# liamscarlett/slate-d35

Measured on AMD Instinct MI355X. Metric: fp64 TFLOP/s (whole node) for dgemm / dpotrf / dgetrf / dgeqrf, n=64k, at 1/2/4/8 MI355X, higher is better.
Workload: dtype fp64

## Files before the change

### csrc/include/slate_amd/local_blas.hh

```
#pragma once

#include <string>
#include <utility>
#include <vector>

#include "types.hh"
#include "comm.hh"
#include "device.hh"

namespace slate {
namespace lb {

struct Ctx {
    Target target = Target::HostTask;
    hipStream_t stream = nullptr;
    bool dev() const { return target == Target::Devices; }
    Loc loc() const { return dev() ? Loc::Device : Loc::Host; }
    static Ctx host() { return Ctx{Target::HostTask, nullptr}; }
    static Ctx device(int queue) { return Ctx{Target::Devices, device::queue(queue)}; }
    Ctx on(int queue) const { return dev() ? device(queue) : *this; }
};

class Scratch {
public:
// ... 42 lines not shown

constexpr int64_t kSkinnyRhs = 16;

template <typename T>
void gemv(Ctx const& c, Op opA, int64_t m, int64_t k, int64_t nr, T alpha, T const* A, int64_t lda, T const* X,
          int64_t ldx, T beta, T* Y, int64_t ldy);

template <typename T>
void gemm_tri(Ctx const& c, Uplo uplo, Op opA, Op opB, int64_t n, int64_t k, T alpha,
              T const* A, int64_t lda, T const* B, int64_t ldb, T beta, T* C, int64_t ldc);

template <typename T>
void herk(Ctx const& c, Uplo uplo, Op op, int64_t n, int64_t k, real_type<T> alpha,
          T const* A, int64_t lda, real_type<T> beta, T* C, int64_t ldc);
template <typename T>
void syrk(Ctx const& c, Uplo uplo, Op op, int64_t n, int64_t k, T alpha,
          T const* A, int64_t lda, T beta, T* C, int64_t ldc);
template <typename T>
void her2k(Ctx const& c, Uplo uplo, Op op, int64_t n, int64_t k, T alpha, T const* A, int64_t lda,
           T const* B, int64_t ldb, real_type<T> beta, T* C, int64_t ldc);
template <typename T>
void syr2k(Ctx const& c, Uplo uplo, Op op, int64_t n, int64_t k, T alpha, T const* A, int64_t lda,
           T const* B, int64_t ldb, T beta, T* C, int64_t ldc);
template <typename T>
void hemm(Ctx const& c, Side side, Uplo uplo, int64_t m, int64_t n, T alpha, T const* A, int64_t lda,
          T const* B, int64_t ldb, T beta, T* C, int64_t ldc, bool hermitian = true);
template <typename T>
void trsm(Ctx const& c, Side side, Uplo uplo, Op op, Diag diag, int64_t m, int64_t n, T alpha,
          T const* A, int64_t lda, T* B, int64_t ldb);
template <typename T>
// ... 59 lines not shown
```

### csrc/include/slate_amd/slate.hh

```
#pragma once

#include "enums.hh"
#include "types.hh"
#include "exception.hh"
#include "util.hh"
#include "device.hh"
#include "comm.hh"
#include "grid.hh"
#include "matrix.hh"
#include "inproc.hh"
#include "func.hh"
#include "method.hh"
#include "matgen.hh"
#include "init.hh"
#include "eig_host.hh"
#include "debug.hh"

#include <vector>

namespace slate {

template <typename T>
using TriangularFactors = std::vector<Matrix<T>>;

// ... 311 lines not shown
GebrdStats gebrd_stats();

template <typename T>
void geqp3(Matrix<T>& A, std::vector<int64_t>& jpvt, TriangularFactors<T>& T_, Options const& opts = {});
template <typename T>
void unmqr_geqp3(Side side, Op op, Matrix<T>& A, TriangularFactors<T>& T_, Matrix<T>& C, Options const& opts = {});
template <typename T>
int64_t gelsy(Matrix<T>& A, Matrix<T>& BX, real_type<T> rcond, Options const& opts = {});
struct Geqp3Stats {
    int64_t columns = 0, panels = 0, host_syncs = 0, norm_recomputes = 0;
    int64_t launches_norms = 0, launches_pivot = 0, launches_swap = 0, launches_column = 0, launches_larfg = 0,
            launches_product = 0, launches_finish = 0, launches_recompute = 0;
    double ms_pivot = 0, ms_product = 0, ms_panel = 0, ms_gemm = 0, ms_larft = 0;
};
Geqp3Stats geqp3_stats();

template <typename T>
void syev(SymmetricMatrix<T>& A, std::vector<real_type<T>>& Lambda, Matrix<T>& Z, Options const& opts = {});
template <typename T>
void sygst(int64_t itype, SymmetricMatrix<T>& A, SymmetricMatrix<T> const& B, Options const& opts = {});
template <typename T>
void sygv(int64_t itype, SymmetricMatrix<T>& A, SymmetricMatrix<T>& B, std::vector<real_type<T>>& Lambda,
          Matrix<T>& Z, Options const& opts = {});
template <typename T>
int64_t sytrf(SymmetricMatrix<T>& A, std::vector<int64_t>& ipiv, Options const& opts = {});
template <typename T>
void sytrs(SymmetricMatrix<T> const& A, std::vector<int64_t> const& ipiv, Matrix<T>& B, Options const& opts = {});
template <typename T>
int64_t sysv(SymmetricMatrix<T>& A, std::vector<int64_t>& ipiv, Matrix<T>& B, Options const& opts = {});
template <typename T>
// ... 23 lines not shown
```

### csrc/kernels/gemm_mfma.hip

```cpp
#include "device_common.hh"
#include "kernels.hh"

#include <cstdarg>
#include <cstdio>
#include <cstdlib>
#include <type_traits>

#ifndef GEMM_SPLIT
#define GEMM_SPLIT 1
#endif
#ifndef GEMM_JB
#define GEMM_JB 2
#endif
#ifndef GEMM_ROT
#define GEMM_ROT true
#endif

namespace slate_amd {
namespace dev {

namespace {
std::atomic<GemmVariantCounter*> g_variant_head{nullptr};
}
GemmVariantCounter::GemmVariantCounter(const char* fmt, ...) {
// ... 450 lines not shown
{
    if (m <= 0 || n <= 0 || batch <= 0) return;
    bool a_kc = (transA != 'N'), b_kc = (transB == 'N');
    if (a_kc && b_kc)
        launch_gemm<T, true, true>(m, n, k, alpha, A, lda, sA, B, ldb, sB, beta, C, ldc, sC, batch, stream);
    else if (a_kc)
        launch_gemm<T, true, false>(m, n, k, alpha, A, lda, sA, B, ldb, sB, beta, C, ldc, sC, batch, stream);
    else if (b_kc)
        launch_gemm<T, false, true>(m, n, k, alpha, A, lda, sA, B, ldb, sB, beta, C, ldc, sC, batch, stream);
    else
        launch_gemm<T, false, false>(m, n, k, alpha, A, lda, sA, B, ldb, sB, beta, C, ldc, sC, batch, stream);
}

template <typename T>
void gemm_tri_real(char uplo, char transA, char transB, int64_t n, int64_t k,
                   T alpha, const T* A, int64_t lda, const T* B, int64_t ldb,
                   T beta, T* C, int64_t ldc, hipStream_t stream)
{
    if (n <= 0) return;
    bool a_kc = (transA != 'N'), b_kc = (transB == 'N');
#define SLATE_TRI_LAUNCH(U)                                                                   \
    if (a_kc && b_kc) launch_gemm<T, true, true, U>(n, n, k, alpha, A, lda, 0, B, ldb, 0, beta, C, ldc, 0, 1, stream); \
    else if (a_kc)    launch_gemm<T, true, false, U>(n, n, k, alpha, A, lda, 0, B, ldb, 0, beta, C, ldc, 0, 1, stream); \
    else if (b_kc)    launch_gemm<T, false, true, U>(n, n, k, alpha, A, lda, 0, B, ldb, 0, beta, C, ldc, 0, 1, stream); \
    else              launch_gemm<T, false, false, U>(n, n, k, alpha, A, lda, 0, B, ldb, 0, beta, C, ldc, 0, 1, stream);
    if (uplo == 'L') { SLATE_TRI_LAUNCH('L') }
    else { SLATE_TRI_LAUNCH('U') }
#undef SLATE_TRI_LAUNCH
}

template <typename T>
void gemm_stair_real(int64_t m, int64_t n, int64_t k, T alpha, const T* A, int64_t lda, const T* B, int64_t ldb,
                     StairMap const& sm, T beta, T* C, int64_t ldc, hipStream_t stream)
{
    if (m <= 0 || n <= 0) return;
    constexpr int VEC = 16 / sizeof(T);
    auto al = [](const void* p) { return (reinterpret_cast<uintptr_t>(p) % 16) == 0; };
    bool aligned = al(A) && al(B) && (lda % VEC == 0) && (ldb % VEC == 0) && sm.nb % VEC == 0;
    launch_tile<T, false, false, 'S', 128, 128>(m, n, k, alpha, A, lda, 0, B, ldb, 0, beta, C, ldc, 0, 1,
                                                aligned, stream, sm);
// ... 19 lines not shown
        s2 += p[(b + 2) * mn];
        s3 += p[(b + 3) * mn];
    }
    for (; b < splits; ++b) s0 += p[b * mn];
    T s = (s0 + s1) + (s2 + s3);
    T* c = C + i + j * ldc;
    *c = (beta == T(0)) ? alpha * s : alpha * s + beta * (*c);
}

template <typename T>
void splitk_reduce(int64_t m, int64_t n, int splits, const T* P, T alpha, T beta, T* C, int64_t ldc, hipStream_t s) {
    if (m <= 0 || n <= 0) return;
    dim3 grid((unsigned)((m + 255) / 256), (unsigned)n);
    hipLaunchKernelGGL(splitk_reduce_kernel<T>, grid, dim3(256), 0, s, m, n, splits, P, alpha, beta, C, ldc);
}
template void splitk_reduce<double>(int64_t, int64_t, int, const double*, double, double, double*, int64_t, hipStream_t);
template void splitk_reduce<float>(int64_t, int64_t, int, const float*, float, float, float*, int64_t, hipStream_t);

template void gemm_tri_real<double>(char, char, char, int64_t, int64_t, double, const double*, int64_t,
                                    const double*, int64_t, double, double*, int64_t, hipStream_t);
template void gemm_tri_real<float>(char, char, char, int64_t, int64_t, float, const float*, int64_t,
                                   const float*, int64_t, float, float*, int64_t, hipStream_t);

template void gemm_real<double>(char, char, int64_t, int64_t, int64_t, double, const double*, int64_t, int64_t,
                                const double*, int64_t, int64_t, double, double*, int64_t, int64_t, int64_t, hipStream_t);
template void gemm_real<float>(char, char, int64_t, int64_t, int64_t, float, const float*, int64_t, int64_t,
                               const float*, int64_t, int64_t, float, float*, int64_t, int64_t, int64_t, hipStream_t);

}
}
```

### csrc/kernels/kernels.hh

```
#pragma once

#include <hip/hip_runtime_api.h>
#include <atomic>
#include <cstdint>
#include "dev_types.hh"
#include "matgen_entry.hh"
#include "slate_amd/secular.hh"
#include "slate_amd/sturm.hh"

namespace slate_amd {
namespace dev {

template <typename T> using rt = typename real_type_t<T>::type;

struct RowDist {
    int64_t row0;
    int64_t mb;
    int64_t lrow_begin;
    int p, rsrc, myrow, rrel;
};
SLATE_HD inline int rd_owner(RowDist const& d, int64_t gr) { return int(((d.row0 + gr) / d.mb + d.rsrc) % d.p); }
SLATE_HD inline int64_t rd_lrow(RowDist const& d, int64_t gr) {
    int64_t R = d.row0 + gr;
    return (R / d.mb / d.p) * d.mb + R % d.mb - d.lrow_begin;
// ... 261 lines not shown
struct GemmVariantCounter {
    char name[56];
    std::atomic<uint64_t> count{0};
    GemmVariantCounter* next = nullptr;
    explicit GemmVariantCounter(const char* fmt, ...) __attribute__((format(printf, 2, 3)));
    void hit() { count.fetch_add(1, std::memory_order_relaxed); }
};
void gemm_variant_counts(void (*fn)(const char* name, uint64_t count, void* arg), void* arg);
template <typename T>
void gemm_real(char transA, char transB, int64_t m, int64_t n, int64_t k,
               T alpha, const T* A, int64_t lda, int64_t sA,
               const T* B, int64_t ldb, int64_t sB,
               T beta, T* C, int64_t ldc, int64_t sC, int64_t batch, hipStream_t stream);
template <typename T>
void gemm_tri_real(char uplo, char transA, char transB, int64_t n, int64_t k,
                   T alpha, const T* A, int64_t lda, const T* B, int64_t ldb,
                   T beta, T* C, int64_t ldc, hipStream_t stream);
template <typename T>
void splitk_reduce(int64_t m, int64_t n, int splits, const T* P, T alpha, T beta, T* C, int64_t ldc, hipStream_t s);
struct StairMap {
    const int64_t* btab = nullptr;
    int64_t c0 = 0, r0 = 0;
    int nb = 0, p = 1, q = 1, prow = 0, pcol = 0;
};
template <typename T>
void gemm_stair_real(int64_t m, int64_t n, int64_t k, T alpha, const T* A, int64_t lda, const T* B, int64_t ldb,
                     StairMap const& sm, T beta, T* C, int64_t ldc, hipStream_t stream);
void gemm_bf16s(int nsplit, char uplo, char transA, char transB, int64_t m, int64_t n, int64_t k,
                float alpha, const float* A, int64_t lda, const float* B, int64_t ldb,
                float beta, float* C, int64_t ldc, hipStream_t stream);
template <typename T>
void gemm_cplx(char uplo, char transA, char transB, int64_t m, int64_t n, int64_t k,
               T alpha, const T* A, int64_t lda, const T* B, int64_t ldb,
               T beta, T* C, int64_t ldc, hipStream_t stream);
// ... 112 lines not shown
```

### csrc/python/bind.cc

```cpp
#include <pybind11/pybind11.h>
#include <chrono>
#include <thread>
#include <pybind11/numpy.h>
#include <pybind11/stl.h>
#include <pybind11/functional.h>

#include "slate_amd/slate.hh"
#include "../src/lu_dist.hh"
#include "slate_amd/trace.hh"
#include "slate_amd/runtime.hh"
#include "slate_amd/inproc.hh"
#include "bind_drivers.hh"
#include <pybind11/numpy.h>

#include <algorithm>
#include <cmath>
#include <complex>
#include <chrono>
#include <cstring>

namespace py = pybind11;
using namespace slate;

class PyHostComm : public HostComm {
// ... 562 lines not shown
        r["host_syncs"] = st.host_syncs;
        r["launches_column"] = st.launches_column;
        r["launches_larfg_u"] = st.launches_larfg_u;
        r["launches_pass1"] = st.launches_pass1;
        r["launches_finish_y"] = st.launches_finish_y;
        r["launches_larfg_v"] = st.launches_larfg_v;
        r["launches_pass2"] = st.launches_pass2;
        r["launches_finish_x"] = st.launches_finish_x;
        r["ms_pass1"] = st.ms_pass1;
        r["ms_pass2"] = st.ms_pass2;
        r["ms_panel"] = st.ms_panel;
        r["ms_gemm"] = st.ms_gemm;
        r["ms_larft"] = st.ms_larft;
        return r;
    });
    m.def("geqp3_stats", []() {
        const Geqp3Stats st = geqp3_stats();
        py::dict r;
        r["columns"] = st.columns;
        r["panels"] = st.panels;
        r["host_syncs"] = st.host_syncs;
        r["norm_recomputes"] = st.norm_recomputes;
        r["launches_norms"] = st.launches_norms;
        r["launches_pivot"] = st.launches_pivot;
        r["launches_swap"] = st.launches_swap;
        r["launches_column"] = st.launches_column;
        r["launches_larfg"] = st.launches_larfg;
        r["launches_product"] = st.launches_product;
        r["launches_finish"] = st.launches_finish;
        r["launches_recompute"] = st.launches_recompute;
// ... 186 lines not shown
```

### csrc/python/bind_drivers.hh

```
#pragma once

#include <pybind11/pybind11.h>
#include <pybind11/stl.h>
#include "slate_amd/slate.hh"
#include "slate_amd/local_blas.hh"
#include "slate_amd/eig_host.hh"
#include <pybind11/numpy.h>

namespace py = pybind11;

slate::Options to_options(py::dict d);

inline int& ops_queue() { static int q = 0; return q; }

template <typename T>
void bind_drivers(py::module_& m, std::string const& s) {
    using namespace slate;
    using R = real_type<T>;
    using G = py::call_guard<py::gil_scoped_release>;
    auto O = [](py::dict d) { return to_options(d); };
    (void)O;
#define DEF(name, ...) m.def((std::string(name) + "_" + s).c_str(), __VA_ARGS__)

    DEF("gemm", [](T a, Matrix<T> const& A, Matrix<T> const& B, T b, Matrix<T>& C, py::dict o) {
// ... 365 lines not shown
    });
    DEF("lb_gemm", [=](std::string ta, std::string tb, int64_t mm, int64_t n, int64_t k, T a, uintptr_t A, int64_t lda,
                       uintptr_t B, int64_t ldb, T b, uintptr_t C, int64_t ldc) {
        py::gil_scoped_release r;
        auto c = dctx();
        lb::gemm<T>(c, cop(ta), cop(tb), mm, n, k, a, (T*)A, lda, (T*)B, ldb, b, (T*)C, ldc);
        dsync(c);
    });
    DEF("lb_herk", [=](std::string up, std::string op, int64_t n, int64_t k, R a, uintptr_t A, int64_t lda, R b,
                       uintptr_t C, int64_t ldc) {
        py::gil_scoped_release r;
        auto c = dctx();
        lb::herk<T>(c, cup(up), cop(op), n, k, a, (T*)A, lda, b, (T*)C, ldc);
        dsync(c);
    });
    DEF("lb_gemm_tri", [=](std::string up, std::string ta, std::string tb, int64_t n, int64_t k, T a, uintptr_t A,
                           int64_t lda, uintptr_t B, int64_t ldb, T b, uintptr_t C, int64_t ldc) {
        py::gil_scoped_release r;
        auto c = dctx();
        lb::gemm_tri<T>(c, cup(up), cop(ta), cop(tb), n, k, a, (T*)A, lda, (T*)B, ldb, b, (T*)C, ldc);
        dsync(c);
    });
    DEF("lb_trsm", [=](std::string sd, std::string up, std::string op, std::string dg, int64_t mm, int64_t n, T a,
                       uintptr_t A, int64_t lda, uintptr_t B, int64_t ldb) {
        py::gil_scoped_release r;
        auto c = dctx();
        lb::trsm<T>(c, sd == "L" ? Side::Left : Side::Right, cup(up), cop(op), dg == "U" ? Diag::Unit : Diag::NonUnit,
                    mm, n, a, (T*)A, lda, (T*)B, ldb);
        dsync(c);
    });
// ... 69 lines not shown
```

### csrc/src/local_blas.cc

```cpp
#include "slate_amd/local_blas.hh"
#include "slate_amd/host_blas.hh"
#include "../kernels/kernels.hh"
#include "slate_amd/eig_host.hh"

#include <atomic>
#include <map>
#include <mutex>
#include <cstring>
#include <cstdlib>

namespace slate {
namespace lb {

using slate_amd::dev::dptr;
using slate_amd::dev::dval;
namespace kd = slate_amd::dev;

namespace {

struct Arena {
    struct Chunk { char* p; size_t size; };
    std::vector<Chunk> chunks;
    size_t cur = 0;
    size_t off = 0;
// ... 223 lines not shown
            return;
        }
        static const int64_t kchunk = [] {
            const char* e = std::getenv("SLATE_GEMM_KCHUNK");
            return e ? std::max<int64_t>(0, std::atoll(e)) : int64_t(0);
        }();
        const bool chunk = kchunk > 0 && k > kchunk && m * n >= int64_t(4096) * 4096;
        for (int64_t k0 = 0; k0 < std::max<int64_t>(k, 1); k0 += chunk ? kchunk : std::max<int64_t>(k, 1)) {
            const int64_t kk = chunk ? std::min(kchunk, k - k0) : k;
            T const* Ak = A + (ta == 'N' ? k0 * lda : k0);
            T const* Bk = B + (tb == 'N' ? k0 : k0 * ldb);
            const T bk = k0 == 0 ? beta : T(1);
            if (uplo == 'G') kd::gemm_real<T>(ta, tb, m, n, kk, alpha, Ak, lda, 0, Bk, ldb, 0, bk, C, ldc, 0, 1, s);
            else {
                slate_assert(m == n);
                kd::gemm_tri_real<T>(uplo, ta, tb, n, kk, alpha, Ak, lda, Bk, ldb, bk, C, ldc, s);
            }
        }
    } else {
        kd::gemm_cplx(uplo, opc(opA), opc(opB), m, n, k, dval(alpha), dptr(A), lda, dptr(B), ldb,
                      dval(beta), dptr(C), ldc, s);
    }
}

template <typename T>
void dset(hipStream_t s, char uplo, int64_t m, int64_t n, T off, T diag, T* A, int64_t lda) {
    kd::geset(uplo, m, n, dval(off), dval(diag), dptr(A), lda, s);
}

template <typename T>
void dcopy(hipStream_t s, int64_t m, int64_t n, T const* A, int64_t lda, T* B, int64_t ldb) {
// ... 73 lines not shown
void real_diag(Ctx const& c, int64_t n, T* C, int64_t ldc) {
    if constexpr (is_complex_v<T>)
        kd::gen_diag('R', 0.0, n, n, dptr(C), ldc, n, 1, 0, 0, 0, n, 1, 0, 0, 0, c.stream);
}
}

template <typename T>
void herk(Ctx const& c, Uplo uplo, Op op, int64_t n, int64_t k, real_type<T> alpha,
          T const* A, int64_t lda, real_type<T> beta, T* C, int64_t ldc) {
    if (n <= 0) return;
    if (!c.dev()) { host::rankk(true, uplo, op, n, k, T(alpha), A, lda, T(beta), C, ldc); return; }
    Op o1 = op == Op::NoTrans ? Op::NoTrans : Op::ConjTrans;
    Op o2 = op == Op::NoTrans ? Op::ConjTrans : Op::NoTrans;
    gemm_tri(c, uplo, o1, o2, n, k, T(alpha), A, lda, A, lda, T(beta), C, ldc);
    real_diag(c, n, C, ldc);
}

template <typename T>
void syrk(Ctx const& c, Uplo uplo, Op op, int64_t n, int64_t k, T alpha,
          T const* A, int64_t lda, T beta, T* C, int64_t ldc) {
    if (n <= 0) return;
    if (!c.dev()) { host::rankk(false, uplo, op, n, k, alpha, A, lda, beta, C, ldc); return; }
    Op o1 = op == Op::NoTrans ? Op::NoTrans : Op::Trans;
    Op o2 = op == Op::NoTrans ? Op::Trans : Op::NoTrans;
    gemm_tri(c, uplo, o1, o2, n, k, alpha, A, lda, A, lda, beta, C, ldc);
}

template <typename T>
void her2k(Ctx const& c, Uplo uplo, Op op, int64_t n, int64_t k, T alpha, T const* A, int64_t lda,
           T const* B, int64_t ldb, real_type<T> beta, T* C, int64_t ldc) {
// ... 781 lines not shown
void copy2d(Ctx const& c, int64_t m, int64_t n, T const* src, int64_t lds, T* dst, int64_t ldd) {
    if (m <= 0 || n <= 0) return;
    if (!c.dev()) {
        for (int64_t j = 0; j < n; ++j) std::memcpy(dst + j * ldd, src + j * lds, m * sizeof(T));
        return;
    }
    device::memcpy2d_async(dst, ldd * sizeof(T), src, lds * sizeof(T), m * sizeof(T), n, c.stream);
}

#define SLATE_LB_INST(T)                                                                                   \
    template void gemm<T>(Ctx const&, Op, Op, int64_t, int64_t, int64_t, T, T const*, int64_t, T const*, int64_t, T, T*, int64_t); \
    template void gemm_tri<T>(Ctx const&, Uplo, Op, Op, int64_t, int64_t, T, T const*, int64_t, T const*, int64_t, T, T*, int64_t); \
    template void gemv<T>(Ctx const&, Op, int64_t, int64_t, int64_t, T, T const*, int64_t, T const*, int64_t, T, T*, int64_t); \
    template void gemm_splitk<T>(Ctx const&, Op, Op, int64_t, int64_t, int64_t, int64_t, T, T const*, int64_t, T const*, int64_t, T, T*, int64_t); \
    template void herk<T>(Ctx const&, Uplo, Op, int64_t, int64_t, real_type<T>, T const*, int64_t, real_type<T>, T*, int64_t); \
    template void syrk<T>(Ctx const&, Uplo, Op, int64_t, int64_t, T, T const*, int64_t, T, T*, int64_t);  \
    template void her2k<T>(Ctx const&, Uplo, Op, int64_t, int64_t, T, T const*, int64_t, T const*, int64_t, real_type<T>, T*, int64_t); \
    template void syr2k<T>(Ctx const&, Uplo, Op, int64_t, int64_t, T, T const*, int64_t, T const*, int64_t, T, T*, int64_t); \
    template void hemm<T>(Ctx const&, Side, Uplo, int64_t, int64_t, T, T const*, int64_t, T const*, int64_t, T, T*, int64_t, bool); \
    template void trsm<T>(Ctx const&, Side, Uplo, Op, Diag, int64_t, int64_t, T, T const*, int64_t, T*, int64_t); \
    template void trmm<T>(Ctx const&, Side, Uplo, Op, Diag, int64_t, int64_t, T, T const*, int64_t, T*, int64_t); \
    template void potrf<T>(Ctx const&, Uplo, int64_t, T*, int64_t, int*, int64_t);                        \
    template void trtri<T>(Ctx const&, Uplo, Diag, int64_t, T*, int64_t);                                 \
    template void trtri_to<T>(Ctx const&, Uplo, Diag, int64_t, T const*, int64_t, T*, int64_t);           \
    template void lauum<T>(Ctx const&, Uplo, int64_t, T*, int64_t);                                        \
    template void getrf_panel<T>(Ctx const&, int64_t, int64_t, T*, int64_t, int64_t*, int64_t*, int*, int64_t, bool, bool, double); \
    template void apply_perm<T>(Ctx const&, int64_t, int64_t const*, int64_t const*, int64_t, T*, int64_t); \
    template void geqrf_panel<T>(Ctx const&, int64_t, int64_t, T*, int64_t, T*, T*, int64_t);             \
    template void larfb<T>(Ctx const&, Side, Op, int64_t, int64_t, int64_t, T const*, int64_t, T const*, int64_t, T*, int64_t); \
    template void form_v<T>(Ctx const&, int64_t, int64_t, T const*, int64_t, T*, int64_t);                \
// ... 54 lines not shown
```

### csrc/src/qr.cc

```cpp
#include "internal.hh"
#include "spread.hh"
#include "lu_dist.hh"

#include <cstdlib>

namespace slate {

using namespace internal;

namespace {

inline int64_t qr_kchunk() {
    static int64_t v = [] {
        const char* e = std::getenv("SLATE_QR_KCHUNK");
        return e ? std::atoll(e) : int64_t(8192);
    }();
    return v;
}

template <typename T>
struct TsqrPanel {
    static constexpr int maxr = 8;
    int64_t nb;
    Work<T> Tloc, Rcur, Rrecv, Ecur, Etmp, Qloc, LUb, Ytmp, Dg, Tw, sgn, taul, Gq;
    Work<int> cq_flag;
    Work<double> cq_ssq;
    int* cq_host = nullptr;
    bool cholqr_on = false;
    std::vector<Work<T>> Sst, Ttt;
    const int64_t tSel = Sched::tok(30, 0);

    TsqrPanel(Target target, int np, int64_t nb_, int64_t max_rows, bool single_cholqr = false) : nb(nb_) {
        if (np <= 1 && !single_cholqr) return;
// ... 22 lines not shown
    TsqrPanel(TsqrPanel const&) = delete;
    TsqrPanel& operator=(TsqrPanel const&) = delete;

    bool cholqr(Sched& S, int qP, Comm& cm, T* ap, int64_t lda, int64_t mr, int64_t kb, int64_t M, int64_t tPan,
                bool shifted) {
        using R = real_type<T>;
        const double u = double(std::numeric_limits<R>::epsilon()) / 2;
        const double shift = 11.0 * (double(M) * double(kb) + double(kb) * double(kb + 1)) * u;
        const Op cT = is_complex_v<T> ? Op::ConjTrans : Op::Trans;
        S.task(qP, {tPan}, {tSel}, [&, ap, mr, kb, shift, shifted, cT](lb::Ctx const& c) {
            trace::Block t2("geqrf_cholqr");
            using DT = slate_amd::dev::dev_t<T>;
            const int64_t ldq = std::max<int64_t>(mr, 1);
            int* dflag = cq_flag.data();
            const int npass = shifted ? 3 : 2;
            lb::copy2d(c, mr, kb, ap, lda, Qloc.data(), ldq);
            if (c.dev()) device::memset_async(dflag + 1, 0, sizeof(int), c.stream);
            else dflag[1] = 0;
            for (int pass = 0; pass < npass; ++pass) {
                T* G = Gq.data();
                lb::herk(c, Uplo::Lower, Op::ConjTrans, kb, mr, R(1), Qloc.data(), ldq, R(0), G, kb);
                cm.allreduce(G, size_t(kb * kb), ReduceOp::Sum, c.loc(), c.stream);
                const bool sh = shifted && pass == 0, chk = pass == npass - 1;
                if (c.dev()) {
                    if (sh) slate_amd::dev::cholqr_shift<DT>(slate_amd::dev::dptr(G), kb, int(kb), shift, c.stream);
                    if (chk)
                        slate_amd::dev::cholqr_check<DT>(slate_amd::dev::dptr(G), kb, int(kb), 0.5, dflag,
                                                         cq_ssq.data(), c.stream);
                } else if (sh) {
                    R tr = 0;
                    for (int64_t i = 0; i < kb; ++i) tr += std::real(G[i + i * kb]);
                    for (int64_t i = 0; i < kb; ++i) G[i + i * kb] += T(R(shift) * tr);
                } else if (chk) {
                    double ssq = 0;
                    for (int64_t j = 0; j < kb; ++j)
                        for (int64_t i = j; i < kb; ++i) {
                            const double d = double(std::abs(G[i + j * kb] - (i == j ? T(1) : T(0))));
                            ssq += (i == j ? 1.0 : 2.0) * d * d;
                        }
                    dflag[0] = (ssq <= 0.25) ? 0 : 1;
                }
                lb::potrf(c, Uplo::Lower, kb, G, kb, dflag + 1, 0);
                lb::trsm(c, Side::Right, Uplo::Lower, cT, Diag::NonUnit, mr, kb, T(1), G, kb, Qloc.data(), ldq);
                if (pass == 0) {
                    lb::set(c, Uplo::General, kb, kb, T(0), T(0), Rcur.data(), kb);
                    lb::copy<T, T>(c, Uplo::Upper, cT, kb, kb, G, kb, Rcur.data(), kb);
                } else {
                    lb::trmm(c, Side::Left, Uplo::Lower, cT, Diag::NonUnit, kb, kb, T(1), G, kb, Rcur.data(), kb);
                }
            }
            if (c.dev()) device::memcpy_async(cq_host, dflag, 2 * sizeof(int), c.stream);
        });
        if (dev_) slate_hip_call(hipStreamSynchronize(S.ctx(qP).stream));
        return cq_host[0] == 0 && cq_host[1] == 0;
    }

    void enqueue(Sched& S, int qP, Comm& cm, int root, int me, std::vector<int64_t> const& rows_r, T* ap,
                 int64_t lda, int64_t mr, int64_t kb, int64_t kd, T* Tk, int64_t tPan, int64_t tP) {
        int64_t Mtot = 0;
        for (auto r : rows_r) Mtot += r;
        if (cholqr_on && kd == kb && Mtot >= 2 * kb &&
            (cholqr(S, qP, cm, ap, lda, mr, kb, Mtot, tPan, false) ||
             cholqr(S, qP, cm, ap, lda, mr, kb, Mtot, tPan, true))) {
            reconstruct(S, qP, cm, root, me, ap, lda, mr, kb, kd, Tk, tPan, tP);
            return;
        }
        tree(S, qP, cm, root, me, rows_r, ap, lda, mr, kb, kd, tPan);
        reconstruct(S, qP, cm, root, me, ap, lda, mr, kb, kd, Tk, tPan, tP);
    }

    void tree(Sched& S, int qP, Comm& cm, int root, int me, std::vector<int64_t> const& rows_r, T* ap,
              int64_t lda, int64_t mr, int64_t kb, int64_t kd, int64_t tPan) {
        const int p = int(rows_r.size());
        const int pk = root;
        const bool diag = (me == root);
        const int myrow = me;
        Comm& colF = cm;
        std::vector<int> part;
        for (int d = 0; d < p; ++d) { int r = (pk + d) % p; if (rows_r[r] > 0) part.push_back(r); }
        const int np = int(part.size());
        std::vector<int64_t> cnt(np);
        for (int i = 0; i < np; ++i) cnt[i] = std::min(rows_r[part[i]], kb);
        int ix = -1;
// ... 83 lines not shown
                S.task(qP, {}, {tSel}, [&, r_, ms, kd](lb::Ctx const& c) {
                    lb::copy2d(c, r_.mine, kd, Etmp.data(), ms, Ecur.data(), r_.mine);
                });
                ecnt = r_.mine;
            }
            S.task(qP, {tSel}, {tSel}, [&, ap, mr, rr, kd, ecnt](lb::Ctx const& c) {
                trace::Block t2("geqrf_tsqr_qlocal");
                lb::set(c, Uplo::General, mr, kd, T(0), T(0), Qloc.data(), mr);
                lb::copy2d(c, ecnt, kd, Ecur.data(), ecnt, Qloc.data(), mr);
                lb::larfb(c, Side::Left, Op::NoTrans, mr, kd, rr, ap, lda, Tloc.data(), nb, Qloc.data(), mr);
            });
        }
    }

    void reconstruct(Sched& S, int qP, Comm& cm, int root, int me, T* ap, int64_t lda, int64_t mr, int64_t kb,
                     int64_t kd, T* Tk, int64_t tPan, int64_t tP) {
        const int pk = root;
        const bool diag = (me == root);
        Comm& colF = cm;
        if (diag) {
            S.task(qP, {tSel}, {tSel}, [&, mr, kd](lb::Ctx const& c) {
                trace::Block t2("geqrf_tsqr_hr_lu");
                lb::add(c, Uplo::General, kd, kd, T(-1), Qloc.data(), mr, T(0), LUb.data(), kd);
                internal::ludist::lu_sign(c, kd, LUb.data(), kd, sgn.data());
            });
        }
        S.task(qP, {}, {tSel}, [&, kd, pk](lb::Ctx const& c) {
            trace::Block t2("geqrf_tsqr_bcast_lu");
            bcast(colF, LUb.data(), size_t(kd * kd), pk, c);
            bcast(colF, sgn.data(), size_t(kd), pk, c);
        });
        const int64_t off = diag ? kd : 0, nbelow = std::max<int64_t>(mr - off, 0);
        S.task(qP, {tSel}, {tPan, tSel}, [&, ap, mr, kd, off, nbelow](lb::Ctx const& c) {
            trace::Block t2("geqrf_tsqr_hr_v");
            lb::trsm(c, Side::Right, Uplo::Upper, Op::NoTrans, Diag::NonUnit, nbelow, kd, T(-1), LUb.data(), kd,
                     Qloc.data() + off, std::max<int64_t>(mr, 1));
            lb::copy2d(c, nbelow, kd, Qloc.data() + off, std::max<int64_t>(mr, 1), ap + off, lda);
        });
        if (diag) {
            S.task(qP, {tSel}, {tPan, tSel, tP}, [&, ap, kb, kd, Tk](lb::Ctx const& c) {
                trace::Block t2("geqrf_tsqr_hr_t");
                lb::set(c, Uplo::General, kd, kd, T(0), T(0), Dg.data(), kd);
                lb::copy2d(c, int64_t(1), kd, sgn.data(), int64_t(1), Dg.data(), kd + 1);
                lb::gemm(c, Op::NoTrans, Op::NoTrans, kd, kb, kd, T(1), Dg.data(), kd, Rcur.data(), kd, T(0), ap,
                         lda);
                lb::copy2d(c, kd, kd, LUb.data(), kd, Ytmp.data(), kd);
                lb::set(c, Uplo::Upper, kd, kd, T(0), T(0), Ytmp.data(), kd);
                lb::add(c, Uplo::Lower, kd, kd, T(1), Ytmp.data(), kd, T(1), ap, lda);
                lb::set(c, Uplo::General, kd, kd, T(0), T(0), Tw.data(), kd);
                lb::copy<T, T>(c, Uplo::Upper, Op::NoTrans, kd, kd, LUb.data(), kd, Tw.data(), kd);
                lb::set(c, Uplo::General, kb, kb, T(0), T(0), Tk, kb);
// ... 10 lines not shown
    const int p = g.p(), q = g.q(), myrow = g.myrow(), mycol = g.mycol();
    const Loc loc = loc_of(target);
    const int64_t mt = A.mt(), nt = A.nt(), m = A.m();
    const int64_t kt = std::min(mt, nt);
    const int64_t nb = A.nb();
    LocalBlock<T> L = A.local(loc, true);
    T* a = L.ptr;
    const int64_t lda = L.ld, mloc = L.m, nloc = L.n;
    LocalBlock<T> LT = Tf.local(loc, true);
    T* tm = LT.ptr;
    const int64_t ldt = LT.ld;
    const int qC = device::kCommQueue, qP = 1;
    Comm& colF = g.col_fast();
    Comm& rowF = g.row_fast();

    Sched S(target);
    const int R = int(std::max<int64_t>(2, la + 2));
    std::vector<Work<T>> WV(R), WT(R), WW(R), WW2(R), Wtau(R);
    for (int r = 0; r < R; ++r) {
        WV[r].resize(target, size_t(std::max<int64_t>(mloc, 1)) * nb);
        WT[r].resize(target, size_t(nb) * nb);
        WW[r].resize(target, size_t(nb) * std::max<int64_t>(nloc, 1));
        WW2[r].resize(target, size_t(nb) * std::max<int64_t>(nloc, 1));
        Wtau[r].resize(target, size_t(nb));
    }
    static const bool cq1_env = [] {
        const char* e = std::getenv("SLATE_QR_CHOLQR1");
        return !e || std::atoi(e) != 0;
    }();
    const bool cq1 = p == 1 && cq1_env && target == Target::Devices && nb >= 256 && A.m() >= 16384;
// ... 247 lines not shown
            trace::Block t2("unmqr_allreduce");
            if (mC > 0) g.row().allreduce(W, W, size_t(ldw * kb), scalar_type<T>(), ReduceOp::Sum, c.loc(), c.stream);
        });
        S.task(0, {tV}, {tC}, [&, kb, Vc, W, W2, Tk](lb::Ctx const& c) {
            trace::Block t2("unmqr_c");
            if (mC <= 0) return;
            lb::gemm(c, Op::NoTrans, op == Op::NoTrans ? Op::NoTrans : cT, mC, kb, kb, T(1), W, ldw, Tk, LT.ld, T(0), W2,
                     ldw);
            lb::gemm(c, Op::NoTrans, cT, mC, ncC, kb, T(-1), W2, ldw, Vc, ldv, T(1), LC.ptr, LC.ld);
        });
    }
    S.wait_all();
    C.storage()->update_origin();
}

}

template <typename T>
void geqrf(Matrix<T>& A, TriangularFactors<T>& T_, Options const& opts) {
    if (auto grp = internal::multi_group<T>({&A})) {
        std::vector<TriangularFactors<T>> Tr(grp->size());
        internal::spread<T>(opts, {{&A, true}}, [&](std::vector<Matrix<T>>& M, int r) {
            geqrf(M[0], Tr[r], opts);
        }, false);
        T_ = internal::factors_from_parts(grp, Tr);
        return;
    }
    if (A.arbitrary_layout()) {
        Matrix<T> Ab = internal::block_cyclic(A, opts);
        geqrf(Ab, T_, opts);
// ... 493 lines not shown
```

### slate_d35_amd/ops/__init__.py

```python
from __future__ import annotations

from .. import _slate

__all__ = ["have_native_ops", "gemm", "gemm_async", "gemm_lowprec", "lowprec_gemm_calls", "bdsdc_stats", "sturm_count", "stebz_stats", "symv_lower", "hetrd_stats", "gebrd_stats", "geqp3_stats", "gemv_t_block", "gemv_n_block", "herk", "gemm_tri", "gemm_variant_counts", "trsm", "potrf", "getrf_panel", "geqrf_panel", "lu_sign",
           "set_queue", "queue_sync"]


def set_queue(q: int):
    _slate.set_ops_queue(q)


def queue_sync(q: int):
    _slate.queue_sync(q)


def have_native_ops() -> bool:
    return hasattr(_slate, "lb_gemm_d")


def _suffix(t):
    import torch
    return {torch.float32: "s", torch.float64: "d", torch.complex64: "c", torch.complex128: "z"}[t.dtype]


# ... 61 lines not shown
        torch.cuda.current_stream(x.device).synchronize()
    y = torch.empty(m, dtype=A.dtype, device=A.device)
    torch.cuda.current_stream(A.device).synchronize()
    if m > 0:
        _slate.lb_symv_lower(_suffix(A), m, pa + (offset + offset * lda) * A.element_size(), lda, x.data_ptr(),
                             y.data_ptr(), repeat)
    return y


def gebrd_stats() -> dict:
    return _slate.gebrd_stats()


def geqp3_stats() -> dict:
    return _slate.geqp3_stats()


def _gemv_block(trans, A, x, row_offset, col_offset, repeat, use_lb):
    import torch
    pa, rows, cols, lda = _cm(A)
    mr, nc = rows - row_offset, cols - col_offset
    assert 0 <= row_offset and 0 <= col_offset and mr >= 0 and nc >= 0
    assert x.numel() == (mr if trans else nc) and x.dtype == A.dtype and x.is_contiguous()
    if x.is_cuda:
        torch.cuda.current_stream(x.device).synchronize()
    y = torch.empty(nc if trans else mr, dtype=A.dtype, device=A.device)
    torch.cuda.current_stream(A.device).synchronize()
    if mr > 0 and nc > 0:
        _slate.lb_gemv_block(_suffix(A), trans, mr, nc, pa + (row_offset + col_offset * lda) * A.element_size(), lda,
                             x.data_ptr(), y.data_ptr(), repeat, use_lb)
# ... 73 lines not shown
```

Before: 63.79.

## Use split-K batched Gram and skip final full-height TRSM in CholQR panel

```diff
diff --git a/csrc/include/slate_amd/local_blas.hh b/csrc/include/slate_amd/local_blas.hh
--- a/csrc/include/slate_amd/local_blas.hh
+++ b/csrc/include/slate_amd/local_blas.hh
@@ -80,6 +80,8 @@
 void herk(Ctx const& c, Uplo uplo, Op op, int64_t n, int64_t k, real_type<T> alpha,
           T const* A, int64_t lda, real_type<T> beta, T* C, int64_t ldc);
 template <typename T>
+int64_t gram_splitk(Ctx const& c, Uplo uplo, int64_t n, int64_t k, T const* A, int64_t lda, T* C, int64_t ldc);
+template <typename T>
 void syrk(Ctx const& c, Uplo uplo, Op op, int64_t n, int64_t k, T alpha,
           T const* A, int64_t lda, T beta, T* C, int64_t ldc);
 template <typename T>
diff --git a/csrc/include/slate_amd/slate.hh b/csrc/include/slate_amd/slate.hh
--- a/csrc/include/slate_amd/slate.hh
+++ b/csrc/include/slate_amd/slate.hh
@@ -349,6 +349,10 @@
     double ms_pivot = 0, ms_product = 0, ms_panel = 0, ms_gemm = 0, ms_larft = 0;
 };
 Geqp3Stats geqp3_stats();
+struct QrPanelStats {
+    int64_t panels_cholqr = 0, gram_calls = 0, gram_tiles = 0, full_height_solves = 0, scale_passes = 0;
+};
+QrPanelStats qr_panel_stats();
 
 template <typename T>
 void syev(SymmetricMatrix<T>& A, std::vector<real_type<T>>& Lambda, Matrix<T>& Z, Options const& opts = {});
diff --git a/csrc/kernels/gemm_mfma.hip b/csrc/kernels/gemm_mfma.hip
--- a/csrc/kernels/gemm_mfma.hip
+++ b/csrc/kernels/gemm_mfma.hip
@@ -488,16 +488,16 @@
 
 template <typename T>
 void gemm_tri_real(char uplo, char transA, char transB, int64_t n, int64_t k,
-                   T alpha, const T* A, int64_t lda, const T* B, int64_t ldb,
-                   T beta, T* C, int64_t ldc, hipStream_t stream)
+                   T alpha, const T* A, int64_t lda, int64_t sA, const T* B, int64_t ldb, int64_t sB,
+                   T beta, T* C, int64_t ldc, int64_t sC, int64_t batch, hipStream_t stream)
 {
-    if (n <= 0) return;
+    if (n <= 0 || batch <= 0) return;
     bool a_kc = (transA != 'N'), b_kc = (transB == 'N');
 #define SLATE_TRI_LAUNCH(U)                                                                   \
-    if (a_kc && b_kc) launch_gemm<T, true, true, U>(n, n, k, alpha, A, lda, 0, B, ldb, 0, beta, C, ldc, 0, 1, stream); \
-    else if (a_kc)    launch_gemm<T, true, false, U>(n, n, k, alpha, A, lda, 0, B, ldb, 0, beta, C, ldc, 0, 1, stream); \
-    else if (b_kc)    launch_gemm<T, false, true, U>(n, n, k, alpha, A, lda, 0, B, ldb, 0, beta, C, ldc, 0, 1, stream); \
-    else              launch_gemm<T, false, false, U>(n, n, k, alpha, A, lda, 0, B, ldb, 0, beta, C, ldc, 0, 1, stream);
+    if (a_kc && b_kc) launch_gemm<T, true, true, U>(n, n, k, alpha, A, lda, sA, B, ldb, sB, beta, C, ldc, sC, batch, stream); \
+    else if (a_kc)    launch_gemm<T, true, false, U>(n, n, k, alpha, A, lda, sA, B, ldb, sB, beta, C, ldc, sC, batch, stream); \
+    else if (b_kc)    launch_gemm<T, false, true, U>(n, n, k, alpha, A, lda, sA, B, ldb, sB, beta, C, ldc, sC, batch, stream); \
+    else              launch_gemm<T, false, false, U>(n, n, k, alpha, A, lda, sA, B, ldb, sB, beta, C, ldc, sC, batch, stream);
     if (uplo == 'L') { SLATE_TRI_LAUNCH('L') }
     else { SLATE_TRI_LAUNCH('U') }
 #undef SLATE_TRI_LAUNCH
@@ -547,13 +547,46 @@
     dim3 grid((unsigned)((m + 255) / 256), (unsigned)n);
     hipLaunchKernelGGL(splitk_reduce_kernel<T>, grid, dim3(256), 0, s, m, n, splits, P, alpha, beta, C, ldc);
 }
+template <typename T>
+__global__ void splitk_reduce_tri_kernel(char uplo, int64_t n, int splits, const T* __restrict__ P,
+                                         T* __restrict__ C, int64_t ldc) {
+    const int64_t i = blockIdx.x * (int64_t)blockDim.x + threadIdx.x;
+    const int64_t j = blockIdx.y;
+    if (i >= n || (uplo == 'L' ? i < j : i > j)) return;
+    T s0 = 0, s1 = 0, s2 = 0, s3 = 0;
+    const int64_t nn = n * n;
+    const T* p = P + i + j * n;
+    int b = 0;
+    for (; b + 4 <= splits; b += 4) {
+        s0 += p[(b + 0) * nn];
+        s1 += p[(b + 1) * nn];
+        s2 += p[(b + 2) * nn];
+        s3 += p[(b + 3) * nn];
+    }
+    for (; b < splits; ++b) s0 += p[b * nn];
+    C[i + j * ldc] = (s0 + s1) + (s2 + s3);
+}
+
+template <typename T>
+void splitk_reduce_tri(char uplo, int64_t n, int splits, const T* P, T* C, int64_t ldc, hipStream_t s) {
+    if (n <= 0) return;
+    dim3 grid((unsigned)((n + 255) / 256), (unsigned)n);
+    hipLaunchKernelGGL(splitk_reduce_tri_kernel<T>, grid, dim3(256), 0, s, uplo, n, splits, P, C, ldc);
+}
+template void splitk_reduce_tri<double>(char, int64_t, int, const double*, double*, int64_t, hipStream_t);
+template void splitk_reduce_tri<float>(char, int64_t, int, const float*, float*, int64_t, hipStream_t);
+
+bool gemm_tri_small_tiles(int64_t n, int64_t batch) { return small_tiles(n, n, batch, true); }
+
 template void splitk_reduce<double>(int64_t, int64_t, int, const double*, double, double, double*, int64_t, hipStream_t);
 template void splitk_reduce<float>(int64_t, int64_t, int, const float*, float, float, float*, int64_t, hipStream_t);
 
-template void gemm_tri_real<double>(char, char, char, int64_t, int64_t, double, const double*, int64_t,
-                                    const double*, int64_t, double, double*, int64_t, hipStream_t);
-template void gemm_tri_real<float>(char, char, char, int64_t, int64_t, float, const float*, int64_t,
-                                   const float*, int64_t, float, float*, int64_t, hipStream_t);
+template void gemm_tri_real<double>(char, char, char, int64_t, int64_t, double, const double*, int64_t, int64_t,
+                                    const double*, int64_t, int64_t, double, double*, int64_t, int64_t, int64_t,
+                                    hipStream_t);
+template void gemm_tri_real<float>(char, char, char, int64_t, int64_t, float, const float*, int64_t, int64_t,
+                                   const float*, int64_t, int64_t, float, float*, int64_t, int64_t, int64_t,
+                                   hipStream_t);
 
 template void gemm_real<double>(char, char, int64_t, int64_t, int64_t, double, const double*, int64_t, int64_t,
                                 const double*, int64_t, int64_t, double, double*, int64_t, int64_t, int64_t, hipStream_t);
diff --git a/csrc/kernels/kernels.hh b/csrc/kernels/kernels.hh
--- a/csrc/kernels/kernels.hh
+++ b/csrc/kernels/kernels.hh
@@ -299,10 +299,13 @@
                T beta, T* C, int64_t ldc, int64_t sC, int64_t batch, hipStream_t stream);
 template <typename T>
 void gemm_tri_real(char uplo, char transA, char transB, int64_t n, int64_t k,
-                   T alpha, const T* A, int64_t lda, const T* B, int64_t ldb,
-                   T beta, T* C, int64_t ldc, hipStream_t stream);
+                   T alpha, const T* A, int64_t lda, int64_t sA, const T* B, int64_t ldb, int64_t sB,
+                   T beta, T* C, int64_t ldc, int64_t sC, int64_t batch, hipStream_t stream);
+bool gemm_tri_small_tiles(int64_t n, int64_t batch);
 template <typename T>
 void splitk_reduce(int64_t m, int64_t n, int splits, const T* P, T alpha, T beta, T* C, int64_t ldc, hipStream_t s);
+template <typename T>
+void splitk_reduce_tri(char uplo, int64_t n, int splits, const T* P, T* C, int64_t ldc, hipStream_t s);
 struct StairMap {
     const int64_t* btab = nullptr;
     int64_t c0 = 0, r0 = 0;
diff --git a/csrc/python/bind.cc b/csrc/python/bind.cc
--- a/csrc/python/bind.cc
+++ b/csrc/python/bind.cc
@@ -600,6 +600,16 @@
         r["ms_larft"] = st.ms_larft;
         return r;
     });
+    m.def("qr_panel_stats", []() {
+        const QrPanelStats st = qr_panel_stats();
+        py::dict r;
+        r["panels_cholqr"] = st.panels_cholqr;
+        r["gram_calls"] = st.gram_calls;
+        r["gram_tiles"] = st.gram_tiles;
+        r["full_height_solves"] = st.full_height_solves;
+        r["scale_passes"] = st.scale_passes;
+        return r;
+    });
     m.def("geqp3_stats", []() {
         const Geqp3Stats st = geqp3_stats();
         py::dict r;
diff --git a/csrc/python/bind_drivers.hh b/csrc/python/bind_drivers.hh
--- a/csrc/python/bind_drivers.hh
+++ b/csrc/python/bind_drivers.hh
@@ -403,6 +403,13 @@
         lb::herk<T>(c, cup(up), cop(op), n, k, a, (T*)A, lda, b, (T*)C, ldc);
         dsync(c);
     });
+    DEF("lb_gram_splitk", [=](std::string up, int64_t n, int64_t k, uintptr_t A, int64_t lda, uintptr_t C, int64_t ldc) {
+        py::gil_scoped_release r;
+        auto c = dctx();
+        const int64_t wg = lb::gram_splitk<T>(c, cup(up), n, k, (T*)A, lda, (T*)C, ldc);
+        dsync(c);
+        return wg;
+    });
     DEF("lb_gemm_tri", [=](std::string up, std::string ta, std::string tb, int64_t n, int64_t k, T a, uintptr_t A,
                            int64_t lda, uintptr_t B, int64_t ldb, T b, uintptr_t C, int64_t ldc) {
         py::gil_scoped_release r;
diff --git a/csrc/src/local_blas.cc b/csrc/src/local_blas.cc
--- a/csrc/src/local_blas.cc
+++ b/csrc/src/local_blas.cc
@@ -261,7 +261,7 @@
             if (uplo == 'G') kd::gemm_real<T>(ta, tb, m, n, kk, alpha, Ak, lda, 0, Bk, ldb, 0, bk, C, ldc, 0, 1, s);
             else {
                 slate_assert(m == n);
-                kd::gemm_tri_real<T>(uplo, ta, tb, n, kk, alpha, Ak, lda, Bk, ldb, bk, C, ldc, s);
+                kd::gemm_tri_real<T>(uplo, ta, tb, n, kk, alpha, Ak, lda, 0, Bk, ldb, 0, bk, C, ldc, 0, 1, s);
             }
         }
     } else {
@@ -365,6 +365,41 @@
     Op o2 = op == Op::NoTrans ? Op::ConjTrans : Op::NoTrans;
     gemm_tri(c, uplo, o1, o2, n, k, T(alpha), A, lda, A, lda, T(beta), C, ldc);
     real_diag(c, n, C, ldc);
+}
+
+namespace {
+kd::GemmVariantCounter g_route_gram_splitk("gram_splitk");
+}
+
+template <typename T>
+int64_t gram_splitk(Ctx const& c, Uplo uplo, int64_t n, int64_t k, T const* A, int64_t lda, T* C, int64_t ldc) {
+    if (n <= 0) return 0;
+    const int64_t t = ceildiv(n, 128), tiles = t * (t + 1) / 2;
+    if constexpr (is_real_v<T>) {
+        if (c.dev() && k >= 1024 && t > 1) {
+            g_route_gram_splitk.hit();
+            const int64_t full = std::min<int64_t>(63, std::max<int64_t>(2, (512 + tiles / 2) / tiles));
+            const int64_t kc = k / full / 16 * 16;
+            const int64_t slices = full + (k > full * kc);
+            hipStream_t s = c.stream;
+            Scratch sc(c);
+            T* P = sc.alloc<T>(size_t(slices) * n * n);
+            const char up = upc(uplo);
+            if (full > 0)
+                kd::gemm_tri_real<T>(up, 'T', 'N', n, kc, T(1), A, lda, kc, A, lda, kc, T(0), P, n, n * n, full, s);
+            if (full < slices)
+                kd::gemm_tri_real<T>(up, 'T', 'N', n, k - full * kc, T(1), A + full * kc, lda, 0, A + full * kc, lda, 0,
+                                     T(0), P + full * n * n, n, 0, 1, s);
+            kd::splitk_reduce_tri<T>(up, n, int(slices), P, C, ldc, s);
+            if (kd::gemm_tri_small_tiles(n, std::max<int64_t>(full, 1))) {
+                const int64_t t64 = ceildiv(n, 64);
+                return t64 * (t64 + 1) / 2;
+            }
+            return tiles;
+        }
+    }
+    herk(c, uplo, Op::ConjTrans, n, k, real_type<T>(1), A, lda, real_type<T>(0), C, ldc);
+    return c.dev() ? tiles : 0;
 }
 
 template <typename T>
@@ -1176,6 +1211,7 @@
     template void gemv<T>(Ctx const&, Op, int64_t, int64_t, int64_t, T, T const*, int64_t, T const*, int64_t, T, T*, int64_t); \
     template void gemm_splitk<T>(Ctx const&, Op, Op, int64_t, int64_t, int64_t, int64_t, T, T const*, int64_t, T const*, int64_t, T, T*, int64_t); \
     template void herk<T>(Ctx const&, Uplo, Op, int64_t, int64_t, real_type<T>, T const*, int64_t, real_type<T>, T*, int64_t); \
+    template int64_t gram_splitk<T>(Ctx const&, Uplo, int64_t, int64_t, T const*, int64_t, T*, int64_t);    \
     template void syrk<T>(Ctx const&, Uplo, Op, int64_t, int64_t, T, T const*, int64_t, T, T*, int64_t);  \
     template void her2k<T>(Ctx const&, Uplo, Op, int64_t, int64_t, T, T const*, int64_t, T const*, int64_t, real_type<T>, T*, int64_t); \
     template void syr2k<T>(Ctx const&, Uplo, Op, int64_t, int64_t, T, T const*, int64_t, T const*, int64_t, T, T*, int64_t); \
diff --git a/csrc/src/qr.cc b/csrc/src/qr.cc
--- a/csrc/src/qr.cc
+++ b/csrc/src/qr.cc
@@ -2,6 +2,7 @@
 #include "spread.hh"
 #include "lu_dist.hh"
 
+#include <atomic>
 #include <cstdlib>
 
 namespace slate {
@@ -17,6 +18,19 @@
     }();
     return v;
 }
+
+inline bool qr_panel_lean() {
+    static const bool v = [] {
+        const char* e = std::getenv("SLATE_QR_PANEL_LEAN");
+        return e ? std::atoi(e) != 0 : true;
+    }();
+    return v;
+}
+
+struct PanelCounters {
+    std::atomic<int64_t> panels_cholqr{0}, gram_calls{0}, gram_tiles{0}, full_height_solves{0}, scale_passes{0};
+    void reset() { panels_cholqr = 0; gram_calls = 0; gram_tiles = 0; full_height_solves = 0; scale_passes = 0; }
+} g_panel;
 
 template <typename T>
 struct TsqrPanel {
@@ -69,12 +83,21 @@
             const int64_t ldq = std::max<int64_t>(mr, 1);
             int* dflag = cq_flag.data();
             const int npass = shifted ? 3 : 2;
+            const bool lean = qr_panel_lean();
+            const int64_t gt = ceildiv(kb, int64_t(128));
             lb::copy2d(c, mr, kb, ap, lda, Qloc.data(), ldq);
             if (c.dev()) device::memset_async(dflag + 1, 0, sizeof(int), c.stream);
             else dflag[1] = 0;
             for (int pass = 0; pass < npass; ++pass) {
                 T* G = Gq.data();
-                lb::herk(c, Uplo::Lower, Op::ConjTrans, kb, mr, R(1), Qloc.data(), ldq, R(0), G, kb);
+                int64_t wg = 0;
+                if (lean) wg = lb::gram_splitk(c, Uplo::Lower, kb, mr, Qloc.data(), ldq, G, kb);
+                else {
+                    lb::herk(c, Uplo::Lower, Op::ConjTrans, kb, mr, R(1), Qloc.data(), ldq, R(0), G, kb);
+                    if (c.dev()) wg = (!is_complex_v<T> && gt * gt < 128 && mr >= 1024) ? gt * gt : gt * (gt + 1) / 2;
+                }
+                g_panel.gram_calls += 1;
+                g_panel.gram_tiles += wg;
                 cm.allreduce(G, size_t(kb * kb), ReduceOp::Sum, c.loc(), c.stream);
                 const bool sh = shifted && pass == 0, chk = pass == npass - 1;
                 if (c.dev()) {
@@ -96,7 +119,10 @@
                     dflag[0] = (ssq <= 0.25) ? 0 : 1;
                 }
                 lb::potrf(c, Uplo::Lower, kb, G, kb, dflag + 1, 0);
-                lb::trsm(c, Side::Right, Uplo::Lower, cT, Diag::NonUnit, mr, kb, T(1), G, kb, Qloc.data(), ldq);
+                if (!(lean && chk)) {
+                    lb::trsm(c, Side::Right, Uplo::Lower, cT, Diag::NonUnit, mr, kb, T(1), G, kb, Qloc.data(), ldq);
+                    g_panel.full_height_solves += 1;
+                }
                 if (pass == 0) {
                     lb::set(c, Uplo::General, kb, kb, T(0), T(0), Rcur.data(), kb);
                     lb::copy<T, T>(c, Uplo::Upper, cT, kb, kb, G, kb, Rcur.data(), kb);
@@ -117,11 +143,12 @@
         if (cholqr_on && kd == kb && Mtot >= 2 * kb &&
             (cholqr(S, qP, cm, ap, lda, mr, kb, Mtot, tPan, false) ||
              cholqr(S, qP, cm, ap, lda, mr, kb, Mtot, tPan, true))) {
-            reconstruct(S, qP, cm, root, me, ap, lda, mr, kb, kd, Tk, tPan, tP);
+            g_panel.panels_cholqr += 1;
+            reconstruct(S, qP, cm, root, me, ap, lda, mr, kb, kd, Tk, tPan, tP, qr_panel_lean());
             return;
         }
         tree(S, qP, cm, root, me, rows_r, ap, lda, mr, kb, kd, tPan);
-        reconstruct(S, qP, cm, root, me, ap, lda, mr, kb, kd, Tk, tPan, tP);
+        reconstruct(S, qP, cm, root, me, ap, lda, mr, kb, kd, Tk, tPan, tP, false);
     }
 
     void tree(Sched& S, int qP, Comm& cm, int root, int me, std::vector<int64_t> const& rows_r, T* ap,
@@ -235,14 +262,22 @@
     }
 
     void reconstruct(Sched& S, int qP, Comm& cm, int root, int me, T* ap, int64_t lda, int64_t mr, int64_t kb,
-                     int64_t kd, T* Tk, int64_t tPan, int64_t tP) {
+                     int64_t kd, T* Tk, int64_t tPan, int64_t tP, bool haveL) {
         const int pk = root;
         const bool diag = (me == root);
         Comm& colF = cm;
+        const Op cT = is_complex_v<T> ? Op::ConjTrans : Op::Trans;
         if (diag) {
-            S.task(qP, {tSel}, {tSel}, [&, mr, kd](lb::Ctx const& c) {
+            S.task(qP, {tSel}, {tSel}, [&, mr, kb, kd, haveL, cT](lb::Ctx const& c) {
                 trace::Block t2("geqrf_tsqr_hr_lu");
-                lb::add(c, Uplo::General, kd, kd, T(-1), Qloc.data(), mr, T(0), LUb.data(), kd);
+                if (haveL) {
+                    lb::copy2d(c, kd, kb, Qloc.data(), mr, Ytmp.data(), kd);
+                    lb::trsm(c, Side::Right, Uplo::Lower, cT, Diag::NonUnit, kd, kb, T(1), Gq.data(), kb, Ytmp.data(),
+                             kd);
+                    lb::add(c, Uplo::General, kd, kd, T(-1), Ytmp.data(), kd, T(0), LUb.data(), kd);
+                } else {
+                    lb::add(c, Uplo::General, kd, kd, T(-1), Qloc.data(), mr, T(0), LUb.data(), kd);
+                }
                 internal::ludist::lu_sign(c, kd, LUb.data(), kd, sgn.data());
             });
         }
@@ -252,10 +287,20 @@
             bcast(colF, sgn.data(), size_t(kd), pk, c);
         });
         const int64_t off = diag ? kd : 0, nbelow = std::max<int64_t>(mr - off, 0);
-        S.task(qP, {tSel}, {tPan, tSel}, [&, ap, mr, kd, off, nbelow](lb::Ctx const& c) {
+        S.task(qP, {tSel}, {tPan, tSel}, [&, ap, mr, kd, off, nbelow, haveL, cT](lb::Ctx const& c) {
             trace::Block t2("geqrf_tsqr_hr_v");
-            lb::trsm(c, Side::Right, Uplo::Upper, Op::NoTrans, Diag::NonUnit, nbelow, kd, T(-1), LUb.data(), kd,
-                     Qloc.data() + off, std::max<int64_t>(mr, 1));
+            if (haveL) {
+                lb::set(c, Uplo::General, kd, kd, T(0), T(0), Tw.data(), kd);
+                lb::copy<T, T>(c, Uplo::Upper, Op::NoTrans, kd, kd, LUb.data(), kd, Tw.data(), kd);
+                lb::trmm(c, Side::Right, Uplo::Lower, cT, Diag::NonUnit, kd, kd, T(-1), Gq.data(), kd, Tw.data(), kd);
+                lb::trsm(c, Side::Right, Uplo::Upper, Op::NoTrans, Diag::NonUnit, nbelow, kd, T(1), Tw.data(), kd,
+                         Qloc.data() + off, std::max<int64_t>(mr, 1));
+            } else {
+                lb::trsm(c, Side::Right, Uplo::Upper, Op::NoTrans, Diag::NonUnit, nbelow, kd, T(-1), LUb.data(), kd,
+                         Qloc.data() + off, std::max<int64_t>(mr, 1));
+                g_panel.scale_passes += 1;
+            }
+            g_panel.full_height_solves += 1;
             lb::copy2d(c, nbelow, kd, Qloc.data() + off, std::max<int64_t>(mr, 1), ap + off, lda);
         });
         if (diag) {
@@ -296,6 +341,7 @@
     Comm& colF = g.col_fast();
     Comm& rowF = g.row_fast();
 
+    g_panel.reset();
     Sched S(target);
     const int R = int(std::max<int64_t>(2, la + 2));
     std::vector<Work<T>> WV(R), WT(R), WW(R), WW2(R), Wtau(R);
@@ -573,6 +619,16 @@
     C.storage()->update_origin();
 }
 
+}
+
+QrPanelStats qr_panel_stats() {
+    QrPanelStats st;
+    st.panels_cholqr = g_panel.panels_cholqr;
+    st.gram_calls = g_panel.gram_calls;
+    st.gram_tiles = g_panel.gram_tiles;
+    st.full_height_solves = g_panel.full_height_solves;
+    st.scale_passes = g_panel.scale_passes;
+    return st;
 }
 
 template <typename T>
diff --git a/slate_d35_amd/ops/__init__.py b/slate_d35_amd/ops/__init__.py
--- a/slate_d35_amd/ops/__init__.py
+++ b/slate_d35_amd/ops/__init__.py
@@ -2,7 +2,7 @@
 
 from .. import _slate
 
-__all__ = ["have_native_ops", "gemm", "gemm_async", "gemm_lowprec", "lowprec_gemm_calls", "bdsdc_stats", "sturm_count", "stebz_stats", "symv_lower", "hetrd_stats", "gebrd_stats", "geqp3_stats", "gemv_t_block", "gemv_n_block", "herk", "gemm_tri", "gemm_variant_counts", "trsm", "potrf", "getrf_panel", "geqrf_panel", "lu_sign",
+__all__ = ["have_native_ops", "gemm", "gemm_async", "gemm_lowprec", "lowprec_gemm_calls", "bdsdc_stats", "sturm_count", "stebz_stats", "symv_lower", "hetrd_stats", "gebrd_stats", "geqp3_stats", "qr_panel_stats", "gram_splitk", "gemv_t_block", "gemv_n_block", "herk", "gemm_tri", "gemm_variant_counts", "trsm", "potrf", "getrf_panel", "geqrf_panel", "lu_sign",
            "set_queue", "queue_sync"]
 
 
@@ -99,6 +99,18 @@
 
 def geqp3_stats() -> dict:
     return _slate.geqp3_stats()
+
+
+def qr_panel_stats() -> dict:
+    return _slate.qr_panel_stats()
+
+
+def gram_splitk(uplo: str, A, C) -> int:
+    fn = getattr(_slate, f"lb_gram_splitk_{_suffix(C)}")
+    pa, k, n, lda = _cm(A)
+    pc, nc, _, ldc = _cm(C)
+    assert nc == n
+    return fn(uplo, n, k, pa, lda, pc, ldc)
 
 
 def _gemv_block(trans, A, x, row_offset, col_offset, repeat, use_lb):
```

Result: no change. 64.19, median of 6 (+0.6%).
